# fpthink/EPC-Net

Measured on AMD Instinct MI355X. Metric: point-clouds/sec (4096 pts) descriptor extraction, higher is better.
Workload: dtype f16x3; 1 GPU; epc-net inference, batch 64x4096x3 fp32 per GPU, NetVLAD K=64, 256-D output (BASELINE.json configs[1]); num_points=4096, precision=EPC_PRECISION_F32 (include/epcnet.h), weights=seeded random init of the architecture (no checkpoint payloads exist), parallelism=independent clouds sharded over 1 GPU(s), no data-path collective

## Files before the change

epc-net_amd/csrc/block.hip:

```cpp
#include "train_common.h"

#define BLK_WAVES 12
#define BLK_THREADS (64 * BLK_WAVES)
#define BLK_PERSIST_MAX_ROUNDS 4096
#define ST_STRIDE 68
#define BLK_PACK EPC_BLOCK_PACK_FLOATS
#define BLK_PACK_S EPC_BLOCK_PACK_FLOATS_S
#define BLK_LDS_FLOATS (BLK_PACK_S + BLK_WAVES * 32 * ST_STRIDE)


__device__ __forceinline__ void acc_init_bias(f32x16& acc, const float* bias32, int h) {
#pragma unroll
    for (int g = 0; g < 4; ++g) {
        const float4 b = ld4(bias32 + 8 * g + 4 * h);
        acc[4 * g + 0] = b.x;
        acc[4 * g + 1] = b.y;
        acc[4 * g + 2] = b.z;
        acc[4 * g + 3] = b.w;
    }
}

__device__ __forceinline__ void kahan_add(float& sum, float& comp, float v) {
    const float y = v - comp;
    const float t = sum + y;
    comp = (t - sum) - y;
    sum = t;
}

__device__ __forceinline__ void relu16(f32x16& a) {
#pragma unroll
    for (int r = 0; r < 16; ++r) a[r] = fmaxf(a[r], 0.f);
}


__device__ __forceinline__ f16x8 ldfrag_h(const float* p) {
    return __builtin_bit_cast(f16x8, *reinterpret_cast<const u32x4*>(p));
}
__device__ __forceinline__ void layer_s64(const float* lw, const float* lbias, const float* ltinv, const f16x8 (&bh)[4],
                                          const f16x8 (&bl)[4], float inv_row, f32x16 (&acc)[2], int lane) {
    const int h = lane >> 5;
#pragma unroll
    for (int t = 0; t < 2; ++t) {
#pragma unroll
        for (int r = 0; r < 16; ++r) acc[t][r] = 0.f;
#pragma unroll
        for (int s = 0; s < 4; ++s) {
            const f16x8 ah = ldfrag_h(lw + (((t * 4 + s) * 2 + 0) * 64 + lane) * 4);
            const f16x8 al = ldfrag_h(lw + (((t * 4 + s) * 2 + 1) * 64 + lane) * 4);
            acc[t] = mfma_f16(al, bh[s], acc[t]);
            acc[t] = mfma_f16(ah, bl[s], acc[t]);
            acc[t] = mfma_f16(ah, bh[s], acc[t]);
        }
#pragma unroll
        for (int g = 0; g < 4; ++g) {
            const float4 ti = ld4(ltinv + 32 * t + 8 * g + 4 * h), b = ld4(lbias + 32 * t + 8 * g + 4 * h);
            acc[t][4 * g + 0] = __builtin_fmaf(acc[t][4 * g + 0], inv_row * ti.x, b.x);
            acc[t][4 * g + 1] = __builtin_fmaf(acc[t][4 * g + 1], inv_row * ti.y, b.y);
            acc[t][4 * g + 2] = __builtin_fmaf(acc[t][4 * g + 2], inv_row * ti.z, b.z);
            acc[t][4 * g + 3] = __builtin_fmaf(acc[t][4 * g + 3], inv_row * ti.w, b.w);
        }
    }
}

__device__ __forceinline__ void layer_acc64(const float* lw, const float* lbias, const float* ltinv, const f32x16 (&in)[2],
                                            f32x16 (&acc)[2], int lane) {
    float m = 0.f;
#pragma unroll
    for (int t = 0; t < 2; ++t)
#pragma unroll
        for (int r = 0; r < 16; ++r) m = fmaxf(m, fabsf(in[t][r]));
    m = fmaxf(m, __shfl_xor(m, 32));
    float sc, inv_row;
    row_scale_pow2(m, sc, inv_row);
    f16x8 fh[4], fl[4];
#pragma unroll
    for (int st = 0; st < 4; ++st) {
        float v[8];
#pragma unroll
        for (int q = 0; q < 8; ++q) v[q] = in[st >> 1][8 * (st & 1) + q];
        split8_f16s(v, sc, fh[st], fl[st]);
    }
    layer_s64(lw, lbias, ltinv, fh, fl, inv_row, acc, lane);
}

__device__ __forceinline__ void acc_to_stage(float* st, const f32x16 (&acc)[2], int lane) {
    const int j = lane & 31, h = lane >> 5;
#pragma unroll
    for (int t = 0; t < 2; ++t)
#pragma unroll
        for (int g = 0; g < 4; ++g)
            st4(st + j * ST_STRIDE + 32 * t + 8 * g + 4 * h,
                make_float4(acc[t][4 * g], acc[t][4 * g + 1], acc[t][4 * g + 2], acc[t][4 * g + 3]));
}

__device__ __forceinline__ float stage_to_bop(const float* st, f16x8 (&bh)[4], f16x8 (&bl)[4], int lane) {
    const int j = lane & 31, h = lane >> 5;
    float v[4][8];
    float m = 0.f;
#pragma unroll
    for (int s = 0; s < 4; ++s) {
        const float4 a = ld4(st + j * ST_STRIDE + 16 * s + 8 * h), b = ld4(st + j * ST_STRIDE + 16 * s + 8 * h + 4);
        v[s][0] = a.x, v[s][1] = a.y, v[s][2] = a.z, v[s][3] = a.w, v[s][4] = b.x, v[s][5] = b.y, v[s][6] = b.z, v[s][7] = b.w;
#pragma unroll
        for (int q = 0; q < 8; ++q) m = fmaxf(m, fabsf(v[s][q]));
    }
    m = fmaxf(m, __shfl_xor(m, 32));
    float sc, inv_row;
    row_scale_pow2(m, sc, inv_row);
#pragma unroll
    for (int s = 0; s < 4; ++s) split8_f16s(v[s], sc, bh[s], bl[s]);
    return inv_row;
}

__device__ __forceinline__ void load_nb20(const char* lists, unsigned row, int cap, bool u16, int (&nb)[EPC_KNN_SELECT]) {
    static_assert(EPC_KNN_SELECT == 20, "five int4 / two int4 + one int2 per row");
    if (u16) {
        const char* r = lists + (size_t)row * cap * 2;
        const uint4 a = *reinterpret_cast<const uint4*>(r), b = *reinterpret_cast<const uint4*>(r + 16);
        const uint2 c = *reinterpret_cast<const uint2*>(r + 32);
        const unsigned int w[10] = {a.x, a.y, a.z, a.w, b.x, b.y, b.z, b.w, c.x, c.y};
#pragma unroll
        for (int k = 0; k < 10; ++k) {
            nb[2 * k] = (int)(w[k] & 0xffffu);
            nb[2 * k + 1] = (int)(w[k] >> 16);
        }
    } else {
        const int4* il = reinterpret_cast<const int4*>(lists + (size_t)row * cap * 4);
#pragma unroll
        for (int m4 = 0; m4 < EPC_KNN_SELECT / 4; ++m4) {
            const int4 t = il[m4];
            nb[4 * m4] = t.x;
            nb[4 * m4 + 1] = t.y;
            nb[4 * m4 + 2] = t.z;
            nb[4 * m4 + 3] = t.w;
        }
    }
}
__device__ __forceinline__ int list_entry(const void* lists, size_t slot, bool u16) {
    return u16 ? (int)reinterpret_cast<const unsigned short*>(lists)[slot] : reinterpret_cast<const int32_t*>(lists)[slot];
}

__global__ __launch_bounds__(BLK_THREADS) void proxyconv_block_kernel(
    const float* __restrict__ x, const float* __restrict__ xyz, const void* __restrict__ idx, int idx_u16,
    const int32_t* __restrict__ cnt, const float* __restrict__ kth, int cap, const float* __restrict__ pack,
    int has_next, int total_points, int n, float kdiv, float* __restrict__ out, int out_stride, int out_off,
    float* __restrict__ x_next) {
    extern __shared__ __attribute__((aligned(16))) float lds[];
    __shared__ int s_next_tile;
    const int tid = threadIdx.x, lane = tid & 63, wave = tid >> 6;
    if (tid == 0) s_next_tile = 0;
    for (int o = tid * 4; o < BLK_PACK_S; o += BLK_THREADS * 4) st4(lds + o, ld4(pack + o));
    __syncthreads();
    const float* wa = lds;
    const float* ba = lds + 4096;
    const float* wb = lds + 4160;
    const float* bb = lds + 4160 + 4096;
    const float* wn = lds + 8320;
    const float* bn = lds + 8320 + 4096;
    const float* tia = lds + BLK_PACK;
    const float* tib = tia + 64;
    const float* tin = tia + 128;
    float* st = lds + BLK_PACK_S + wave * 32 * ST_STRIDE;

    const int ntiles = total_points / 32;
    const int nwg = (int)gridDim.x, per = ntiles / nwg, rem = ntiles % nwg;
    auto first_tile_of = [&](int wg) { return wg * per + min(wg, rem); };
    const int xq = nwg >> 3, xr = nwg & 7, xcd = (int)blockIdx.x & 7, slot = (int)blockIdx.x >> 3;
    const int xcd_wgs = xq + (xcd < xr ? 1 : 0);
    const int xcd_first = xcd < xr ? xcd * (xq + 1) : xr * (xq + 1) + (xcd - xr) * xq;
    const int t_begin = first_tile_of(xcd_first), t_end = first_tile_of(xcd_first + xcd_wgs);
    const int p = lane >> 4, q = lane & 15;
    const bool u16 = idx_u16 != 0;
    const float rk = 1.0f / kdiv;
    auto div_k = [&](float a) {
        const float q0 = a * rk;
        return __builtin_fmaf(__builtin_fmaf(-q0, kdiv, a), rk, q0);
    };
  for (;;) {
    int t_draw = 0;
    if (lane == 0) t_draw = atomicAdd(&s_next_tile, 1);
    const int d = __builtin_amdgcn_readfirstlane(t_draw);
    const int tile = t_begin + (d >> 2) * (xcd_wgs * 4) + slot * 4 + (d & 3);
    if (tile >= t_end) break;
    const int g0 = tile * 32;
    const int cloud_base = __builtin_amdgcn_readfirstlane((g0 / n) * n);
    const char* xc = reinterpret_cast<const char*>(x) + (size_t)cloud_base * 256;
    auto row32 = [&](int row) { return *reinterpret_cast<const float4*>(xc + (unsigned)(row * 256 + q * 16)); };
    const int wg0 = __builtin_amdgcn_readfirstlane(g0);

    float4 xm[8];
#pragma unroll
    for (int s = 0; s < 8; ++s) {
        const int g = g0 + 4 * s + p;
        const int c = cnt[g];
        const bool ovf = c > cap;
        float4 acc = make_float4(0.f, 0.f, 0.f, 0.f);
        if (!ovf) {
            int nb[EPC_KNN_SELECT];
            load_nb20(reinterpret_cast<const char*>(idx), (unsigned)(wg0 + 4 * s + p), cap, u16, nb);
            float4 v[EPC_KNN_SELECT];
#pragma unroll
            for (int m = 0; m < EPC_KNN_SELECT; ++m) v[m] = row32(nb[m]);
#pragma unroll
            for (int m = 0; m < EPC_KNN_SELECT; ++m) {
                acc.x += v[m].x;
                acc.y += v[m].y;
                acc.z += v[m].z;
                acc.w += v[m].w;
            }
            for (int m = EPC_KNN_SELECT; m < c; ++m) {
                const float4 w = row32(list_entry(idx, (size_t)g * cap + m, u16));
                acc.x += w.x;
                acc.y += w.y;
                acc.z += w.z;
                acc.w += w.w;
            }
        }
        if (__any(ovf)) {
            if (ovf) {
                const float* pc = xyz + (size_t)cloud_base * 3;
                const int i = g - cloud_base;
                const float xi = pc[3 * i], yi = pc[3 * i + 1], zi = pc[3 * i + 2];
                const float sqi = sq3(xi, yi, zi);
                const float kv = kth[g];
                float4 comp = make_float4(0.f, 0.f, 0.f, 0.f);
                for (int j = 0; j < n; ++j) {
                    const float xj = pc[3 * j], yj = pc[3 * j + 1], zj = pc[3 * j + 2];
                    const float a = neg_sq_dist(sqi, xi, yi, zi, xj, yj, zj, sq3(xj, yj, zj));
                    if (a >= kv) {
                        const float4 w = row32(j);
                        kahan_add(acc.x, comp.x, w.x);
                        kahan_add(acc.y, comp.y, w.y);
                        kahan_add(acc.z, comp.z, w.z);
                        kahan_add(acc.w, comp.w, w.w);
                    }
                }
            }
        }
        acc.x = div_k(acc.x), acc.y = div_k(acc.y), acc.z = div_k(acc.z), acc.w = div_k(acc.w);
        xm[s] = acc;
        const float4 xi4 = row32(g - cloud_base);
        st4(st + (4 * s + p) * ST_STRIDE + 4 * q,
            make_float4(acc.x - xi4.x, acc.y - xi4.y, acc.z - xi4.z, acc.w - xi4.w));
    }

    f16x8 bh[4], bl[4];
    f32x16 a1[2], a2[2];
    float inv_row = stage_to_bop(st, bh, bl, lane);
    layer_s64(wa, ba, tia, bh, bl, inv_row, a1, lane);
    relu16(a1[0]);
    relu16(a1[1]);
    layer_acc64(wb, bb, tib, a1, a2, lane);
    relu16(a2[0]);
    relu16(a2[1]);

    acc_to_stage(st, a2, lane);
#pragma unroll
    for (int s = 0; s < 8; ++s) {
        float* row = st + (4 * s + p) * ST_STRIDE + 4 * q;
        const float4 t = ld4(row);
        const float4 o = make_float4(t.x + xm[s].x, t.y + xm[s].y, t.z + xm[s].z, t.w + xm[s].w);
        st4(out + (size_t)(g0 + 4 * s + p) * out_stride + out_off + 4 * q, o);
        st4(row, o);
    }
    if (!has_next) continue;

    inv_row = stage_to_bop(st, bh, bl, lane);
    layer_s64(wn, bn, tin, bh, bl, inv_row, a1, lane);
    relu16(a1[0]);
    relu16(a1[1]);
    acc_to_stage(st, a1, lane);
#pragma unroll
    for (int s = 0; s < 8; ++s)
        st4(x_next + (size_t)(g0 + 4 * s + p) * 64 + 4 * q, ld4(st + (4 * s + p) * ST_STRIDE + 4 * q));
  }
}

#define ST16 72


__device__ __forceinline__ void layer_f16(const float* lw, const float* lbias, const f16x8 (&bop)[4], f32x16 (&acc)[2],
                                          int lane) {
    const int h = lane >> 5;
#pragma unroll
    for (int t = 0; t < 2; ++t) {
        acc_init_bias(acc[t], lbias + 32 * t, h);
#pragma unroll
        for (int s = 0; s < 4; ++s) {
            const f16x8 ah = ldfrag16(lw + (((t * 4 + s) * 2 + 0) * 64 + lane) * 4);
            const f16x8 al = ldfrag16(lw + (((t * 4 + s) * 2 + 1) * 64 + lane) * 4);
            acc[t] = mfma_f16(al, bop[s], acc[t]);
            acc[t] = mfma_f16(ah, bop[s], acc[t]);
        }
    }
}

typedef unsigned short u16x2_t __attribute__((ext_vector_type(2)));
__device__ __forceinline__ void range_track(u16x2_t& m, unsigned int packed_pair) {
    m = __builtin_elementwise_max(m, __builtin_bit_cast(u16x2_t, packed_pair & 0x7fff7fffu));
}
__device__ __forceinline__ void range_track4(u16x2_t& m, const u32x4& w) {
    range_track(m, w[0]), range_track(m, w[1]), range_track(m, w[2]), range_track(m, w[3]);
}

__device__ __forceinline__ uint2 relu_descale_pack4(const f32x16& a, int r0) {
    _Float16 hv[4];
#pragma unroll
    for (int e = 0; e < 4; ++e) hv[e] = (_Float16)(fmaxf(a[r0 + e], 0.f) * (1.0f / W5_SCALE));
    uint2 w;
    w.x = (unsigned)__builtin_bit_cast(unsigned short, hv[0]) | ((unsigned)__builtin_bit_cast(unsigned short, hv[1]) << 16);
    w.y = (unsigned)__builtin_bit_cast(unsigned short, hv[2]) | ((unsigned)__builtin_bit_cast(unsigned short, hv[3]) << 16);
    return w;
}

__device__ __forceinline__ void acc_to_stage16(unsigned short* st, const f32x16 (&acc)[2], int lane) {
    const int j = lane & 31, h = lane >> 5;
#pragma unroll
    for (int t = 0; t < 2; ++t)
#pragma unroll
        for (int g = 0; g < 4; ++g)
            *reinterpret_cast<uint2*>(st + j * ST16 + 32 * t + 8 * g + 4 * h) = relu_descale_pack4(acc[t], 4 * g);
}

__device__ __forceinline__ void stage16_to_bop(const unsigned short* st, f16x8 (&bop)[4], int lane) {
    const int j = lane & 31, h = lane >> 5;
#pragma unroll
    for (int s = 0; s < 4; ++s)
        bop[s] = __builtin_bit_cast(f16x8, *reinterpret_cast<const u32x4*>(st + j * ST16 + 16 * s + 8 * h));
}

#define BLK16_WAVES 16
#define BLK16_THREADS (64 * BLK16_WAVES)
#define BLK16_LDS_BYTES (BLK_PACK * 4 + BLK16_WAVES * 32 * ST16 * 2)

__global__ __launch_bounds__(BLK16_THREADS) void proxyconv_block_f16_kernel(
    const unsigned short* __restrict__ x16, const float* __restrict__ xyz, const void* __restrict__ idx, int idx_u16,
    const int32_t* __restrict__ cnt, const float* __restrict__ kth, int cap, const float* __restrict__ pack,
    int has_next, int total_points, int n, float kdiv, unsigned short* __restrict__ out16, int out_stride, int out_off,
    unsigned short* __restrict__ x_next16, int32_t* __restrict__ status) {
    extern __shared__ __attribute__((aligned(16))) float lds[];
    const int tid = threadIdx.x, lane = tid & 63, wave = tid >> 6;
    for (int o = tid * 4; o < BLK_PACK; o += BLK16_THREADS * 4) st4(lds + o, ld4(pack + o));
    __syncthreads();
    const float* wa = lds;
    const float* ba = lds + 4096;
    const float* wb = lds + 4160;
    const float* bb = lds + 4160 + 4096;
    const float* wn = lds + 8320;
    const float* bn = lds + 8320 + 4096;
    unsigned short* st = reinterpret_cast<unsigned short*>(lds + BLK_PACK) + wave * 32 * ST16;

    const int bid = xcd_contiguous_block(blockIdx.x, gridDim.x);
    const int g0 = (bid * BLK16_WAVES + wave) * 32;
    if (g0 >= total_points) return;
    const int cloud_base = __builtin_amdgcn_readfirstlane((g0 / n) * n);
    const int p = lane >> 3, q = lane & 7;
    const char* xc = reinterpret_cast<const char*>(x16) + (size_t)cloud_base * 128;
    auto row16 = [&](int row) { return *reinterpret_cast<const u32x4*>(xc + (unsigned)(row * 128 + q * 16)); };
    auto add_row = [&](float (&acc)[8], const u32x4& raw) {
#pragma unroll
        for (int w2 = 0; w2 < 4; ++w2) {
            asm("v_fma_mix_f32 %0, %1, 1.0, %0 op_sel:[0,0,0] op_sel_hi:[1,0,0]" : "+v"(acc[2 * w2]) : "v"(raw[w2]));
            asm("v_fma_mix_f32 %0, %1, 1.0, %0 op_sel:[1,0,0] op_sel_hi:[1,0,0]" : "+v"(acc[2 * w2 + 1]) : "v"(raw[w2]));
        }
    };
    const int wg0 = __builtin_amdgcn_readfirstlane(g0);
    const bool u16 = idx_u16 != 0;
    const float rk = 1.0f / kdiv;
    auto div_k = [&](float a) {
        const float q0 = a * rk;
        return __builtin_fmaf(__builtin_fmaf(-q0, kdiv, a), rk, q0);
    };

    u16x2_t rmax = {0, 0};
    auto report_range = [&]() {
        const bool over = max(rmax[0], rmax[1]) >= 0x7c00;
        if (status && __builtin_amdgcn_ballot_w64(over) != 0ull && lane == 0) atomicOr(status + g0 / n, EPC_STATUS_FP16_RANGE);
    };
    float xm[4][8];
#pragma unroll
    for (int s = 0; s < 4; ++s) {
        const int g = g0 + 8 * s + p;
        const int c = cnt[g];
        const bool ovf = c > cap;
        float acc[8];
#pragma unroll
        for (int e = 0; e < 8; ++e) acc[e] = 0.f;
        if (!ovf) {
            int nb[EPC_KNN_SELECT];
            load_nb20(reinterpret_cast<const char*>(idx), (unsigned)(wg0 + 8 * s + p), cap, u16, nb);
            u32x4 raw[EPC_KNN_SELECT];
#pragma unroll
            for (int m = 0; m < EPC_KNN_SELECT; ++m) raw[m] = row16(nb[m]);
#pragma unroll
            for (int m = 0; m < EPC_KNN_SELECT; ++m) add_row(acc, raw[m]);
            for (int m = EPC_KNN_SELECT; m < c; ++m) add_row(acc, row16(list_entry(idx, (size_t)g * cap + m, u16)));
        }
        if (__any(ovf)) {
            if (ovf) {
                const float* pc = xyz + (size_t)cloud_base * 3;
                const int i = g - cloud_base;
                const float xi = pc[3 * i], yi = pc[3 * i + 1], zi = pc[3 * i + 2];
                const float sqi = sq3(xi, yi, zi);
                const float kv = kth[g];
                for (int j = 0; j < n; ++j) {
                    const float xj = pc[3 * j], yj = pc[3 * j + 1], zj = pc[3 * j + 2];
                    const float a = neg_sq_dist(sqi, xi, yi, zi, xj, yj, zj, sq3(xj, yj, zj));
                    if (a >= kv) add_row(acc, row16(j));
                }
            }
        }
        const f16x8 self = __builtin_bit_cast(f16x8, row16(g - cloud_base));
        f16x8 t16;
#pragma unroll
        for (int e = 0; e < 8; ++e) {
            xm[s][e] = div_k(acc[e]);
            t16[e] = (_Float16)(xm[s][e] - (float)self[e]);
        }
        const u32x4 tw = __builtin_bit_cast(u32x4, t16);
        range_track4(rmax, tw);
        *reinterpret_cast<u32x4*>(st + (8 * s + p) * ST16 + 8 * q) = tw;
    }

    f16x8 bop[4];
    f32x16 a1[2], a2[2];
    stage16_to_bop(st, bop, lane);
    layer_f16(wa, ba, bop, a1, lane);
    {
#pragma unroll
        for (int k4 = 0; k4 < 4; ++k4) {
            const uint2 lo = relu_descale_pack4(a1[k4 >> 1], 8 * (k4 & 1)), hi = relu_descale_pack4(a1[k4 >> 1], 8 * (k4 & 1) + 4);
            u32x4 w;
            w[0] = lo.x, w[1] = lo.y, w[2] = hi.x, w[3] = hi.y;
            range_track4(rmax, w);
            bop[k4] = __builtin_bit_cast(f16x8, w);
        }
    }
    layer_f16(wb, bb, bop, a2, lane);

    acc_to_stage16(st, a2, lane);
#pragma unroll
    for (int s = 0; s < 4; ++s) {
        unsigned short* row = st + (8 * s + p) * ST16 + 8 * q;
        const u32x4 t16w = *reinterpret_cast<const u32x4*>(row);
        const f16x8 t16 = __builtin_bit_cast(f16x8, t16w);
        f16x8 o16;
#pragma unroll
        for (int e = 0; e < 8; ++e) o16[e] = (_Float16)((float)t16[e] + xm[s][e]);
        const u32x4 ow = __builtin_bit_cast(u32x4, o16);
        range_track4(rmax, t16w);
        range_track4(rmax, ow);
        *reinterpret_cast<u32x4*>(out16 + (size_t)(g0 + 8 * s + p) * out_stride + out_off + 8 * q) = ow;
        *reinterpret_cast<u32x4*>(row) = ow;
    }
    if (!has_next) {
        report_range();
        return;
    }

    stage16_to_bop(st, bop, lane);
    layer_f16(wn, bn, bop, a1, lane);
    acc_to_stage16(st, a1, lane);
#pragma unroll
    for (int s = 0; s < 4; ++s) {
        const u32x4 xw = *reinterpret_cast<const u32x4*>(st + (8 * s + p) * ST16 + 8 * q);
        range_track4(rmax, xw);
        *reinterpret_cast<u32x4*>(x_next16 + (size_t)(g0 + 8 * s + p) * 64 + 8 * q) = xw;
    }
    report_range();
}

__global__ __launch_bounds__(256) void conv1_kernel(const float* __restrict__ xyz, const float* __restrict__ pack,
                                                    int total_points, float* __restrict__ x,
                                                    unsigned short* __restrict__ x16, int32_t* __restrict__ status,
                                                    int n) {
    const int t = blockIdx.x * 256 + threadIdx.x;
    const int g = t >> 4, q = t & 15;
    if (g >= total_points) return;
    const float px = xyz[3 * (size_t)g], py = xyz[3 * (size_t)g + 1], pz = xyz[3 * (size_t)g + 2];
    const float4 w0 = ld4(pack + 4 * q), w1 = ld4(pack + 64 + 4 * q), w2 = ld4(pack + 128 + 4 * q);
    const float4 b = ld4(pack + 192 + 4 * q);
    const float4 y = conv1_quad(px, py, pz, w0, w1, w2, b);
    if (x) st4(x + (size_t)g * 64 + 4 * q, y);
    if (x16) {
        reinterpret_cast<uint2*>(x16)[(size_t)g * 16 + q] = pack_half4(y);
        if (status && fmaxf(fmaxf(y.x, y.y), fmaxf(y.z, y.w)) > 65504.0f) atomicOr(status + g / n, EPC_STATUS_FP16_RANGE);
    }
}

int epc_conv1_launch(const float* xyz, const void* packed_conv1, int num_points_total, float* x, void* x16,
                     int32_t* status, int n, void* stream) {
    EPC_CHECK_ARG(xyz && packed_conv1 && (x || x16), "null pointer");
    EPC_CHECK_ARG(num_points_total >= 0 && (!status || n > 0), "bad shape");
    if (num_points_total == 0) return EPC_OK;
    const long threads = (long)num_points_total * 16;
    hipLaunchKernelGGL(conv1_kernel, dim3((unsigned)((threads + 255) / 256)), dim3(256), 0, (hipStream_t)stream,
                       xyz, (const float*)packed_conv1, num_points_total, x, (unsigned short*)x16, status, n);
    EPC_CHECK_LAUNCH();
    return EPC_OK;
}

extern "C" int epc_conv1_fwd(const float* xyz, const void* packed_conv1, int num_points_total, float* x, void* x16,
                             void* stream) {
    return epc_conv1_launch(xyz, packed_conv1, num_points_total, x, x16, nullptr, 0, stream);
}

extern "C" int epc_proxyconv_block_fwd(const float* x, const void* x16, const float* xyz, const void* idx, int idx_u16,
                                       const int32_t* cnt, const float* kth, int cap, const void* packed_block,
                                       int has_next, int num_clouds, int n, int knn, float* out, void* out16,
                                       int out_stride, int out_off, float* x_next, void* x_next16, int32_t* status,
                                       void* stream) {
    const bool f16 = x16 != nullptr;
    EPC_CHECK_ARG(xyz && idx && cnt && kth && packed_block, "null pointer");
    if (f16) {
        EPC_CHECK_ARG(out16 && (!has_next || x_next16), "fp16 mode needs out16 (and x_next16 when has_next)");
        EPC_CHECK_ARG(out_stride % 8 == 0 && out_off % 8 == 0 && out_off + 64 <= out_stride, "bad output slice");
    } else {
        EPC_CHECK_ARG(x && out && (!has_next || x_next), "f32 mode needs x, out (and x_next when has_next)");
        EPC_CHECK_ARG(out_stride % 4 == 0 && out_off % 4 == 0 && out_off + 64 <= out_stride, "bad output slice");
    }
    EPC_CHECK_ARG(cap == EPC_KNN_CAP, "neighbour-list capacity must be EPC_KNN_CAP (32)");
    EPC_CHECK_ARG(n > 0 && n % 32 == 0, "num_points must be a multiple of 32");
    EPC_CHECK_ARG(knn > 0, "KNN divisor must be positive");
    if (num_clouds <= 0) return num_clouds == 0 ? EPC_OK : EPC_EINVAL;
    const long total = (long)num_clouds * n;
    EPC_CHECK_ARG(total < (1L << 31), "too many points");
    const size_t lds_bytes = f16 ? (size_t)BLK16_LDS_BYTES : BLK_LDS_FLOATS * sizeof(float);
    const void* fn = f16 ? reinterpret_cast<const void*>(proxyconv_block_f16_kernel)
                         : reinterpret_cast<const void*>(proxyconv_block_kernel);
    EPC_SET_DYN_LDS(fn, lds_bytes);
    const int wpb = f16 ? BLK16_WAVES : BLK_WAVES;
    unsigned blocks = (unsigned)((total + wpb * 32 - 1) / (wpb * 32));
    if (!f16) {
        const int num_cus = epc_device_cu_count();
        if (blocks > (unsigned)num_cus && blocks <= (unsigned)BLK_PERSIST_MAX_ROUNDS * (unsigned)num_cus) blocks = (unsigned)num_cus;
    }
    if (f16)
        hipLaunchKernelGGL(proxyconv_block_f16_kernel, dim3(blocks), dim3(BLK16_THREADS), lds_bytes, (hipStream_t)stream,
                           (const unsigned short*)x16, xyz, idx, idx_u16, cnt, kth, cap, (const float*)packed_block, has_next,
                           (int)total, n, (float)knn, (unsigned short*)out16, out_stride, out_off,
                           (unsigned short*)x_next16, status);
    else
        hipLaunchKernelGGL(proxyconv_block_kernel, dim3(blocks), dim3(BLK_THREADS), lds_bytes, (hipStream_t)stream, x,
                           xyz, idx, idx_u16, cnt, kth, cap, (const float*)packed_block, has_next, (int)total, n, (float)knn,
                           out, out_stride, out_off, x_next);
    EPC_CHECK_LAUNCH();
    return EPC_OK;
}
```

epc-net_amd/lib.py:

```python
from __future__ import annotations

import ctypes
import os
import re
from ctypes import POINTER, c_char_p, c_float, c_int, c_int32, c_void_p

import torch

_HERE = os.path.dirname(os.path.abspath(__file__))
LIB_PATH = os.environ.get("EPCNET_LIB") or os.path.join(_HERE, "libepcnet_hip.so")
HEADER_PATH = os.path.join(os.path.dirname(_HERE), "include", "epcnet.h")

_SCALARS = {"int": c_int, "long": ctypes.c_long, "long long": ctypes.c_longlong, "float": c_float,
            "size_t": ctypes.c_size_t, "int32_t": c_int32, "uint32_t": ctypes.c_uint32}
_REVISIT_SCALARS = dict(_SCALARS, double=ctypes.c_double)
_POINTEES = {"float*": torch.float32, "double*": torch.float64, "int32_t*": torch.int32, "int*": torch.int32, "long*": torch.int64}


def parse_header(text: str, need_status: bool = True, scalars=_SCALARS):
    text = re.sub(r"/\*.*?\*/", " ", text, flags=re.S)
    text = re.sub(r"#ifdef __cplusplus.*?#endif", " ", text, flags=re.S)
    constants = {n: int(v, 0) for n, v in re.findall(r"^[ \t]*#[ \t]*define[ \t]+(EPC_\w+)[ \t]+(.*?)[ \t]*$", text, flags=re.M)}
    enum = re.search(r"typedef\s+enum\s+epc_status\s*\{(.*?)\}", text, flags=re.S)
    if not enum and need_status:
        raise ValueError("epcnet.h: no enum epc_status")
    status = {n.strip(): int(v, 0) for n, v in (m.split("=") for m in enum.group(1).split(","))} if enum else {}
    text = re.sub(r"^[ \t]*#.*$", " ", text, flags=re.M)
    text = re.sub(r"typedef\s+(struct|enum)\s+\w+\s*(\{[^{}]*\})?\s*\w+\s*;", " ", text)

    def ctype(t):
        return re.sub(r"\s*\*\s*", "*", " ".join(re.sub(r"\bconst\b", " ", t).split()))

    functions = {}
    for decl in text.split(";"):
        if not decl.strip():
            continue
        m = re.fullmatch(r"\s*([\w\s*]+?)\b(epc(?:net)?_\w+)\s*\((.*)\)\s*", decl, flags=re.S)
        if not m or m.group(2) in functions:
            raise ValueError("epcnet.h: not a declaration, or a second one of its name: %r" % " ".join(decl.split()))
        ret, name, params, names = ctype(m.group(1)), m.group(2), [], []
        if ret not in scalars and ret != "char*":
            raise ValueError("epcnet.h: %s: unknown return type %r" % (name, ret))
        for p in ([] if m.group(3).strip() == "void" else m.group(3).split(",")):
            pm = re.fullmatch(r"\s*(.*[\s*])(\w+)\s*", p, flags=re.S)
            if not pm or (ctype(pm.group(1)) not in scalars and "*" not in pm.group(1)):
                raise ValueError("epcnet.h: %s: unknown parameter type in %r" % (name, " ".join(p.split())))
            params.append(ctype(pm.group(1)))
            names.append(pm.group(2))
        functions[name] = (ret, params, names)
    return functions, constants, status


if not os.path.exists(HEADER_PATH):
    raise ImportError(
        "%s is missing: the binding is derived from the library's header (keep include/ beside the package).  "
        "There is no second copy of the declarations." % HEADER_PATH)
with open(HEADER_PATH) as _f:
    _functions, _constants, _status = parse_header(_f.read())
POSES_HEADER_PATH = os.path.join(os.path.dirname(HEADER_PATH), "epcnet_poses.h")
if not os.path.exists(POSES_HEADER_PATH):
    raise ImportError("%s is missing: the binding of the pose entries is derived from it" % POSES_HEADER_PATH)
with open(POSES_HEADER_PATH) as _f:
    _pose_functions, _pose_constants, _ = parse_header(_f.read(), need_status=False)
if set(_pose_functions) & set(_functions) or set(_pose_constants) & set(_constants):
    raise ImportError("epcnet_poses.h declares a name epcnet.h declares")
_constants.update(_pose_constants)
POSE_EXPORTS = list(_pose_functions)
SCANS_HEADER_PATH = os.path.join(os.path.dirname(HEADER_PATH), "epcnet_scans.h")
if not os.path.exists(SCANS_HEADER_PATH):
    raise ImportError("%s is missing: the binding of the scan entries is derived from it" % SCANS_HEADER_PATH)
with open(SCANS_HEADER_PATH) as _f:
    _scan_functions, _scan_constants, _ = parse_header(_f.read(), need_status=False)
if set(_scan_functions) & (set(_functions) | set(_pose_functions)) or set(_scan_constants) & set(_constants):
    raise ImportError("epcnet_scans.h declares a name epcnet.h or epcnet_poses.h declares")
_constants.update(_scan_constants)
SCAN_EXPORTS = list(_scan_functions)
SUBMAPS_HEADER_PATH = os.path.join(os.path.dirname(HEADER_PATH), "epcnet_submaps.h")
if not os.path.exists(SUBMAPS_HEADER_PATH):
    raise ImportError("%s is missing: the binding of the submap entries is derived from it" % SUBMAPS_HEADER_PATH)
with open(SUBMAPS_HEADER_PATH) as _f:
    _submap_functions, _submap_constants, _ = parse_header(_f.read(), need_status=False)
if (set(_submap_functions) & (set(_functions) | set(_pose_functions) | set(_scan_functions))
        or set(_submap_constants) & set(_constants)):
    raise ImportError("epcnet_submaps.h declares a name an earlier header declares")
_constants.update(_submap_constants)
SUBMAP_EXPORTS = list(_submap_functions)
STAMPS_HEADER_PATH = os.path.join(os.path.dirname(HEADER_PATH), "epcnet_stamps.h")
if not os.path.exists(STAMPS_HEADER_PATH):
    raise ImportError("%s is missing: the binding of the stamp entries is derived from it" % STAMPS_HEADER_PATH)
with open(STAMPS_HEADER_PATH) as _f:
    _stamp_functions, _stamp_constants, _ = parse_header(_f.read(), need_status=False)
if (set(_stamp_functions) & (set(_functions) | set(_pose_functions) | set(_scan_functions) | set(_submap_functions))
        or set(_stamp_constants) & set(_constants)):
    raise ImportError("epcnet_stamps.h declares a name an earlier header declares")
_constants.update(_stamp_constants)
STAMP_EXPORTS = list(_stamp_functions)
REVISITS_HEADER_PATH = os.path.join(os.path.dirname(HEADER_PATH), "epcnet_revisits.h")
if not os.path.exists(REVISITS_HEADER_PATH):
    raise ImportError("%s is missing: the binding of the revisit entries is derived from it" % REVISITS_HEADER_PATH)
with open(REVISITS_HEADER_PATH) as _f:
    _revisit_functions, _revisit_constants, _ = parse_header(_f.read(), need_status=False, scalars=_REVISIT_SCALARS)
if (set(_revisit_functions) & (set(_functions) | set(_pose_functions) | set(_scan_functions) | set(_submap_functions) | set(_stamp_functions))
        or set(_revisit_constants) & set(_constants)):
    raise ImportError("epcnet_revisits.h declares a name an earlier header declares")
_constants.update(_revisit_constants)
REVISIT_EXPORTS = list(_revisit_functions)
PAIRS_HEADER_PATH = os.path.join(os.path.dirname(HEADER_PATH), "epcnet_pairs.h")
if not os.path.exists(PAIRS_HEADER_PATH):
    raise ImportError("%s is missing: the binding of the pair entries is derived from it" % PAIRS_HEADER_PATH)
with open(PAIRS_HEADER_PATH) as _f:
    _pair_functions, _pair_constants, _ = parse_header(_f.read(), need_status=False, scalars=_REVISIT_SCALARS)
if (set(_pair_functions) & (set(_functions) | set(_pose_functions) | set(_scan_functions) | set(_submap_functions) | set(_stamp_functions)
                            | set(_revisit_functions))
        or set(_pair_constants) & set(_constants)):
    raise ImportError("epcnet_pairs.h declares a name an earlier header declares")
_constants.update(_pair_constants)
PAIR_EXPORTS = list(_pair_functions)
globals().update(_constants, **_status)
EXPORTS = list(_functions)
STATUS_NAMES = {v: n for n, v in _status.items()}
PRECISION_IDS = {"f32": _constants["EPC_PRECISION_F32"], "fast": _constants["EPC_PRECISION_FAST"]}
STAGE_NAMES = ["sort", "knn", "conv1", "block1", "block2", "block3", "block4", "conv5", "aggregate", "head"]
assert len(STAGE_NAMES) == _constants["EPC_NUM_STAGES"]


class EpcNetError(RuntimeError):
    def __init__(self, status: int, message: str):
        super().__init__("%s (%d): %s" % (STATUS_NAMES.get(status, "?"), status, message))
        self.status = status


class EpcCfg(ctypes.Structure):
    _fields_ = [("arch", c_int32), ("num_points", c_int32), ("input_dim", c_int32), ("knn", c_int32),
                ("cluster_size", c_int32), ("output_dim", c_int32), ("groups", c_int32),
                ("micro_batch", c_int32), ("precision", c_int32)]


_P = c_void_p


class ChainFwdBlock(ctypes.Structure):
    _fields_ = [(n, _P) for n in ("gamma0", "beta0", "in_bias", "Wa", "ba", "gamma_a", "beta_a", "Wb", "bb", "gamma_b", "beta_b",
                                  "W0_next", "b0_next", "z0", "mean0", "var0", "mean_a", "var_a", "mean_b", "var_b",
                                  "d", "za", "zb", "z0_next")]


class ChainFwdArgs(ctypes.Structure):
    _fields_ = [("blk", ChainFwdBlock * _constants["EPC_CHAIN_MAX_BLOCKS"]), ("nblocks", c_int), ("xyz", _P), ("idx", _P), ("cnt", _P),
                ("kth", _P), ("cap", c_int), ("num_clouds", c_int), ("n", c_int), ("knn", c_int), ("cat", _P), ("cat_bf16", _P),
                ("eps", c_float), ("workspace", _P), ("spin_ticks", ctypes.c_longlong)]


if not os.path.exists(LIB_PATH):
    raise ImportError(
        "%s is missing: build the HIP extension first (python -c 'import __graft_entry__ as g; g.build()' or "
        "make -C epc-net_amd/csrc).  There is no CPU fallback." % LIB_PATH)

_lib = ctypes.CDLL(LIB_PATH)

_POINTERS = {"epc_cfg*": POINTER(EpcCfg), "epc_chain_fwd_args*": POINTER(ChainFwdArgs)}
for _name, (_ret, _params, _) in (list(_functions.items()) + list(_pose_functions.items()) + list(_scan_functions.items())
                                  + list(_submap_functions.items()) + list(_stamp_functions.items()) + list(_revisit_functions.items())
                                  + list(_pair_functions.items())):
    _fn = getattr(_lib, _name)
    _fn.restype = c_char_p if _ret == "char*" else _REVISIT_SCALARS[_ret]
    _fn.argtypes = [_REVISIT_SCALARS.get(_t) or _POINTERS.get(_t, c_void_p) for _t in _params]


def lib() -> ctypes.CDLL:
    return _lib


def check(status: int) -> None:
    if status != _status["EPC_OK"]:
        raise EpcNetError(status, (_lib.epc_last_error() or b"").decode("utf-8", "replace"))


def ptr(t) -> int:
    if t is None:
        return None
    if not t.is_cuda:
        raise EpcNetError(-1, "tensor must live on a ROCm device: the HIP path has no CPU fallback")
    if not t.is_contiguous():
        raise EpcNetError(-1, "tensor must be contiguous")
    return t.data_ptr()


def micro_batch_of(cfg: "EpcCfg", num_clouds: int) -> int:
    mb = cfg.micro_batch if cfg.micro_batch > 0 else (64 if cfg.arch == _constants["EPC_ARCH_EPC_NET"] else 256)
    return max(1, min(int(num_clouds), int(mb)))


def current_stream() -> int:
    return torch.cuda.current_stream().cuda_stream


def _converter(where: str, ctype: str):
    if "*" in ctype:
        dtype = _POINTEES.get(ctype)

        def pointer(a):
            if a is None:
                return None
            try:
                on_device = a.is_cuda
            except AttributeError:
                return a
            if not on_device:
                raise EpcNetError(-1, "%s: tensor must live on a ROCm device: the HIP path has no CPU fallback" % where)
            if dtype is not None and a.dtype is not dtype:
                raise EpcNetError(-1, "%s: the header declares %s there, the tensor is %s" % (where, dtype, a.dtype))
            return a.data_ptr()
        return pointer
    cast = float if ctype in ("float", "double") else int

    def scalar(a):
        if type(a) is cast:
            return a
        if isinstance(a, torch.Tensor):
            raise TypeError("%s: a tensor where the header declares a scalar" % where)
        return cast(a)
    return scalar


def _launcher(name: str, fn, types, names):
    signature = "%s(%s)" % (name, ", ".join("%s %s" % tn for tn in zip(types, names)))
    converters = [_converter("%s: argument %d (%s %s)" % (name, i + 1, t, n), t) for i, (t, n) in enumerate(zip(types[:-1], names))]
    ok = _status["EPC_OK"]

    def launch(*args, stream=None):
        if len(args) != len(converters):
            raise TypeError("%s takes %d arguments and the stream, got %d" % (signature, len(converters), len(args)))
        status = fn(*[c(a) for c, a in zip(converters, args)], current_stream() if stream is None else stream)
        if status != ok:
            check(status)
    launch.__name__ = launch.__qualname__ = name
    launch.__doc__ = signature
    return launch


class run:
    """The checked call form of every LAUNCHING entry point -- one whose last parameter is ``void* stream`` -- by name:
    ``run.epc_col_sum(dy, rows, cout, db, ws, n)`` takes the header's arguments without the stream.  A tensor is legal at a pointer
    parameter only, must live on the device and have the dtype of a typed pointee (``_POINTEES``; anything goes at ``void*``); its
    address is passed, strides are the caller's.  None, an int address and ctypes objects pass unchanged, scalars through int() /
    float().  The stream is the current one (or ``stream=``), the returned status goes through ``check``.  Everything else --
    size queries, ``*_ok``, the forwards whose stream is not last -- is called on the raw handle ``lib()``."""


LAUNCHING = [_n for _n, (_, _t, _pn) in _functions.items() if _t and (_t[-1], _pn[-1]) == ("void*", "stream")]
for _name in LAUNCHING:
    assert _functions[_name][0] == "int", "%s takes a stream and does not return a status" % _name
    setattr(run, _name, staticmethod(_launcher(_name, getattr(_lib, _name), *_functions[_name][1:])))
for _name, (_ret, _t, _pn) in _pose_functions.items():
    assert _ret == "int" and (_t[-1], _pn[-1]) == ("void*", "stream"), "%s does not take a stream last and return a status" % _name
    setattr(run, _name, staticmethod(_launcher(_name, getattr(_lib, _name), _t, _pn)))
for _name, (_ret, _t, _pn) in (list(_scan_functions.items()) + list(_submap_functions.items()) + list(_stamp_functions.items())
                               + list(_revisit_functions.items()) + list(_pair_functions.items())):
    if _t and (_t[-1], _pn[-1]) == ("void*", "stream"):
        assert _ret == "int", "%s takes a stream and does not return a status" % _name
        setattr(run, _name, staticmethod(_launcher(_name, getattr(_lib, _name), _t, _pn)))


def require_gpu() -> None:
    if not torch.cuda.is_available():
        raise EpcNetError(-3, "no ROCm device visible: the EPC-Net HIP path cannot run (no CPU fallback)")
```

Before: 59120 clouds/s.

## Add fast neighbor-gather path with coalesced index staging and software-pipelined gathers

Adds a templated fast path to the fp32 proxy-conv block kernel. When the cap matches the compile-time value and no point in the tile overflows, it loads the tile's neighbor index lists with coalesced wave-wide uint4 loads, parks them in LDS, and software-pipelines the 20-neighbor row gathers so the next row's loads overlap the current sum. Output stores become nontemporal. The old path remains as form 0 behind a new entry point, which adds code size and register pressure.

```diff
diff --git a/epc-net_amd/csrc/block.hip b/epc-net_amd/csrc/block.hip
--- a/epc-net_amd/csrc/block.hip
+++ b/epc-net_amd/csrc/block.hip
@@ -1,4 +1,6 @@
+#include <type_traits>
 #include "train_common.h"
+#include "../../include/epcnet_forms.h"
 
 #define BLK_WAVES 12
 #define BLK_THREADS (64 * BLK_WAVES)
@@ -27,6 +29,12 @@
     sum = t;
 }
 
+__device__ __forceinline__ void st4_stream(float* p, float4 v) {
+    typedef float f32x4_t __attribute__((ext_vector_type(4)));
+    const f32x4_t w = {v.x, v.y, v.z, v.w};
+    __builtin_nontemporal_store(w, reinterpret_cast<f32x4_t*>(p));
+}
+
 __device__ __forceinline__ void relu16(f32x16& a) {
 #pragma unroll
     for (int r = 0; r < 16; ++r) a[r] = fmaxf(a[r], 0.f);
@@ -140,6 +148,30 @@
     return u16 ? (int)reinterpret_cast<const unsigned short*>(lists)[slot] : reinterpret_cast<const int32_t*>(lists)[slot];
 }
 
+template <bool U16>
+struct Nb20Words {
+    unsigned int w[U16 ? EPC_KNN_SELECT / 2 : EPC_KNN_SELECT];
+    __device__ __forceinline__ void load(const float* row) {
+        static_assert(EPC_KNN_SELECT == 20, "five uint4 / two uint4 + one uint2 per row");
+        const uint4* r = reinterpret_cast<const uint4*>(row);
+        if (U16) {
+            const uint4 a = r[0], b = r[1];
+            const uint2 c = *reinterpret_cast<const uint2*>(row + 8);
+            w[0] = a.x, w[1] = a.y, w[2] = a.z, w[3] = a.w, w[4] = b.x, w[5] = b.y, w[6] = b.z, w[7] = b.w, w[8] = c.x, w[9] = c.y;
+        } else {
+#pragma unroll
+            for (int m4 = 0; m4 < EPC_KNN_SELECT / 4; ++m4) {
+                const uint4 t = r[m4];
+                w[4 * m4] = t.x, w[4 * m4 + 1] = t.y, w[4 * m4 + 2] = t.z, w[4 * m4 + 3] = t.w;
+            }
+        }
+    }
+    __device__ __forceinline__ int entry(int m) const {
+        return U16 ? (int)((m & 1) ? w[m >> 1] >> 16 : w[m >> 1] & 0xffffu) : (int)w[m];
+    }
+};
+
+template <int FORM>
 __global__ __launch_bounds__(BLK_THREADS) void proxyconv_block_kernel(
     const float* __restrict__ x, const float* __restrict__ xyz, const void* __restrict__ idx, int idx_u16,
     const int32_t* __restrict__ cnt, const float* __restrict__ kth, int cap, const float* __restrict__ pack,
@@ -176,6 +208,7 @@
         const float q0 = a * rk;
         return __builtin_fmaf(__builtin_fmaf(-q0, kdiv, a), rk, q0);
     };
+    const bool cap_ok = cap == EPC_KNN_CAP;
   for (;;) {
     int t_draw = 0;
     if (lane == 0) t_draw = atomicAdd(&s_next_tile, 1);
@@ -189,6 +222,68 @@
     const int wg0 = __builtin_amdgcn_readfirstlane(g0);
 
     float4 xm[8];
+    int c32 = 0;
+    uint4 l0 = make_uint4(0, 0, 0, 0), l1 = l0;
+    const uint4* lb = reinterpret_cast<const uint4*>(reinterpret_cast<const char*>(idx) +
+                                                     (size_t)tile * (32 * EPC_KNN_CAP) * (u16 ? 2 : 4));
+    if (FORM == 1 && cap_ok) {
+        c32 = cnt[g0 + (lane & 31)];
+        l0 = lb[lane];
+        l1 = lb[64 + lane];
+    }
+    const bool fast = FORM == 1 && cap_ok && !__any(c32 > EPC_KNN_SELECT);
+    auto park = [&](int i, const uint4& w, int rb) {
+        *reinterpret_cast<uint4*>(st + (16 * i / rb) * ST_STRIDE + (16 * i % rb) / 4) = w;
+    };
+    auto fast_passes = [&](auto u16_c) {
+        constexpr bool U16 = decltype(u16_c)::value;
+        constexpr int rb = (U16 ? 2 : 4) * EPC_KNN_CAP;
+        uint4 l2 = l0, l3 = l0;
+        if (!U16) {
+            l2 = lb[128 + lane];
+            l3 = lb[192 + lane];
+        }
+        park(lane, l0, rb);
+        park(64 + lane, l1, rb);
+        Nb20Words<U16> nb;
+        float4 v[EPC_KNN_SELECT];
+        nb.load(st + p * ST_STRIDE);
+        float4 own = row32(g0 + p - cloud_base);
+#pragma unroll
+        for (int m = 0; m < EPC_KNN_SELECT; ++m) v[m] = row32(nb.entry(m));
+        if (!U16) {
+            park(128 + lane, l2, rb);
+            park(192 + lane, l3, rb);
+        }
+#pragma unroll
+        for (int s = 0; s < 8; ++s) {
+            float4 own_n = own;
+            if (s < 7) {
+                nb.load(st + (4 * (s + 1) + p) * ST_STRIDE);
+                own_n = row32(g0 + 4 * (s + 1) + p - cloud_base);
+            }
+            float4 acc = make_float4(0.f, 0.f, 0.f, 0.f);
+#pragma unroll
+            for (int m = 0; m < EPC_KNN_SELECT; ++m) {
+                acc.x += v[m].x;
+                acc.y += v[m].y;
+                acc.z += v[m].z;
+                acc.w += v[m].w;
+                if (s < 7) v[m] = row32(nb.entry(m));
+            }
+            acc.x = div_k(acc.x), acc.y = div_k(acc.y), acc.z = div_k(acc.z), acc.w = div_k(acc.w);
+            xm[s] = acc;
+            st4(st + (4 * s + p) * ST_STRIDE + 4 * q,
+                make_float4(acc.x - own.x, acc.y - own.y, acc.z - own.z, acc.w - own.w));
+            own = own_n;
+        }
+    };
+    if (fast) {
+        if (u16)
+            fast_passes(std::true_type{});
+        else
+            fast_passes(std::false_type{});
+    } else {
 #pragma unroll
     for (int s = 0; s < 8; ++s) {
         const int g = g0 + 4 * s + p;
@@ -243,6 +338,7 @@
         st4(st + (4 * s + p) * ST_STRIDE + 4 * q,
             make_float4(acc.x - xi4.x, acc.y - xi4.y, acc.z - xi4.z, acc.w - xi4.w));
     }
+    }
 
     f16x8 bh[4], bl[4];
     f32x16 a1[2], a2[2];
@@ -260,7 +356,7 @@
         float* row = st + (4 * s + p) * ST_STRIDE + 4 * q;
         const float4 t = ld4(row);
         const float4 o = make_float4(t.x + xm[s].x, t.y + xm[s].y, t.z + xm[s].z, t.w + xm[s].w);
-        st4(out + (size_t)(g0 + 4 * s + p) * out_stride + out_off + 4 * q, o);
+        st4_stream(out + (size_t)(g0 + 4 * s + p) * out_stride + out_off + 4 * q, o);
         st4(row, o);
     }
     if (!has_next) continue;
@@ -505,11 +601,11 @@
     return epc_conv1_launch(xyz, packed_conv1, num_points_total, x, x16, nullptr, 0, stream);
 }
 
-extern "C" int epc_proxyconv_block_fwd(const float* x, const void* x16, const float* xyz, const void* idx, int idx_u16,
-                                       const int32_t* cnt, const float* kth, int cap, const void* packed_block,
-                                       int has_next, int num_clouds, int n, int knn, float* out, void* out16,
-                                       int out_stride, int out_off, float* x_next, void* x_next16, int32_t* status,
-                                       void* stream) {
+static int proxyconv_block_fwd_impl(const float* x, const void* x16, const float* xyz, const void* idx, int idx_u16,
+                                    const int32_t* cnt, const float* kth, int cap, const void* packed_block,
+                                    int has_next, int num_clouds, int n, int knn, float* out, void* out16,
+                                    int out_stride, int out_off, float* x_next, void* x_next16, int32_t* status,
+                                    int form, void* stream) {
     const bool f16 = x16 != nullptr;
     EPC_CHECK_ARG(xyz && idx && cnt && kth && packed_block, "null pointer");
     if (f16) {
@@ -526,8 +622,9 @@
     const long total = (long)num_clouds * n;
     EPC_CHECK_ARG(total < (1L << 31), "too many points");
     const size_t lds_bytes = f16 ? (size_t)BLK16_LDS_BYTES : BLK_LDS_FLOATS * sizeof(float);
+    const auto f32_kernel = form == 0 ? proxyconv_block_kernel<0> : proxyconv_block_kernel<1>;
     const void* fn = f16 ? reinterpret_cast<const void*>(proxyconv_block_f16_kernel)
-                         : reinterpret_cast<const void*>(proxyconv_block_kernel);
+                         : reinterpret_cast<const void*>(f32_kernel);
     EPC_SET_DYN_LDS(fn, lds_bytes);
     const int wpb = f16 ? BLK16_WAVES : BLK_WAVES;
     unsigned blocks = (unsigned)((total + wpb * 32 - 1) / (wpb * 32));
@@ -541,9 +638,27 @@
                            (int)total, n, (float)knn, (unsigned short*)out16, out_stride, out_off,
                            (unsigned short*)x_next16, status);
     else
-        hipLaunchKernelGGL(proxyconv_block_kernel, dim3(blocks), dim3(BLK_THREADS), lds_bytes, (hipStream_t)stream, x,
+        hipLaunchKernelGGL(f32_kernel, dim3(blocks), dim3(BLK_THREADS), lds_bytes, (hipStream_t)stream, x,
                            xyz, idx, idx_u16, cnt, kth, cap, (const float*)packed_block, has_next, (int)total, n, (float)knn,
                            out, out_stride, out_off, x_next);
     EPC_CHECK_LAUNCH();
     return EPC_OK;
 }
+
+extern "C" int epc_proxyconv_block_fwd(const float* x, const void* x16, const float* xyz, const void* idx, int idx_u16,
+                                       const int32_t* cnt, const float* kth, int cap, const void* packed_block,
+                                       int has_next, int num_clouds, int n, int knn, float* out, void* out16,
+                                       int out_stride, int out_off, float* x_next, void* x_next16, int32_t* status,
+                                       void* stream) {
+    return proxyconv_block_fwd_impl(x, x16, xyz, idx, idx_u16, cnt, kth, cap, packed_block, has_next, num_clouds, n, knn, out,
+                                    out16, out_stride, out_off, x_next, x_next16, status, 1, stream);
+}
+
+extern "C" int epcnet_block_fwd_form(const float* x, const void* x16, const float* xyz, const void* idx, int idx_u16,
+                                     const int32_t* cnt, const float* kth, int cap, const void* packed_block, int has_next,
+                                     int num_clouds, int n, int knn, float* out, void* out16, int out_stride, int out_off,
+                                     float* x_next, void* x_next16, int32_t* status, int form, void* stream) {
+    EPC_CHECK_ARG(form == 0 || form == 1, "form 0 or 1");
+    return proxyconv_block_fwd_impl(x, x16, xyz, idx, idx_u16, cnt, kth, cap, packed_block, has_next, num_clouds, n, knn, out,
+                                    out16, out_stride, out_off, x_next, x_next16, status, form, stream);
+}
diff --git a/epc-net_amd/lib.py b/epc-net_amd/lib.py
--- a/epc-net_amd/lib.py
+++ b/epc-net_amd/lib.py
@@ -116,6 +116,17 @@
     raise ImportError("epcnet_pairs.h declares a name an earlier header declares")
 _constants.update(_pair_constants)
 PAIR_EXPORTS = list(_pair_functions)
+FORMS_HEADER_PATH = os.path.join(os.path.dirname(HEADER_PATH), "epcnet_forms.h")
+if not os.path.exists(FORMS_HEADER_PATH):
+    raise ImportError("%s is missing: the binding of the form entries is derived from it" % FORMS_HEADER_PATH)
+with open(FORMS_HEADER_PATH) as _f:
+    _form_functions, _form_constants, _ = parse_header(_f.read(), need_status=False)
+if (set(_form_functions) & (set(_functions) | set(_pose_functions) | set(_scan_functions) | set(_submap_functions) | set(_stamp_functions)
+                            | set(_revisit_functions) | set(_pair_functions))
+        or set(_form_constants) & set(_constants)):
+    raise ImportError("epcnet_forms.h declares a name an earlier header declares")
+_constants.update(_form_constants)
+FORM_EXPORTS = list(_form_functions)
 globals().update(_constants, **_status)
 EXPORTS = list(_functions)
 STATUS_NAMES = {v: n for n, v in _status.items()}
@@ -161,7 +172,7 @@
 _POINTERS = {"epc_cfg*": POINTER(EpcCfg), "epc_chain_fwd_args*": POINTER(ChainFwdArgs)}
 for _name, (_ret, _params, _) in (list(_functions.items()) + list(_pose_functions.items()) + list(_scan_functions.items())
                                   + list(_submap_functions.items()) + list(_stamp_functions.items()) + list(_revisit_functions.items())
-                                  + list(_pair_functions.items())):
+                                  + list(_pair_functions.items()) + list(_form_functions.items())):
     _fn = getattr(_lib, _name)
     _fn.restype = c_char_p if _ret == "char*" else _REVISIT_SCALARS[_ret]
     _fn.argtypes = [_REVISIT_SCALARS.get(_t) or _POINTERS.get(_t, c_void_p) for _t in _params]
@@ -256,7 +267,7 @@
     assert _ret == "int" and (_t[-1], _pn[-1]) == ("void*", "stream"), "%s does not take a stream last and return a status" % _name
     setattr(run, _name, staticmethod(_launcher(_name, getattr(_lib, _name), _t, _pn)))
 for _name, (_ret, _t, _pn) in (list(_scan_functions.items()) + list(_submap_functions.items()) + list(_stamp_functions.items())
-                               + list(_revisit_functions.items()) + list(_pair_functions.items())):
+                               + list(_revisit_functions.items()) + list(_pair_functions.items()) + list(_form_functions.items())):
     if _t and (_t[-1], _pn[-1]) == ("void*", "stream"):
         assert _ret == "int", "%s takes a stream and does not return a status" % _name
         setattr(run, _name, staticmethod(_launcher(_name, getattr(_lib, _name), _t, _pn)))
diff --git a/include/epcnet_forms.h b/include/epcnet_forms.h
--- /dev/null
+++ b/include/epcnet_forms.h
@@ -0,0 +1,19 @@
+#ifndef EPCNET_FORMS_H
+#define EPCNET_FORMS_H
+
+#include <stddef.h>
+#include <stdint.h>
+
+#ifdef __cplusplus
+extern "C" {
+#endif
+
+int epcnet_block_fwd_form(const float* x, const void* x16, const float* xyz, const void* idx, int idx_u16, const int32_t* cnt,
+                          const float* kth, int cap, const void* packed_block, int has_next, int num_clouds, int n, int knn,
+                          float* out, void* out16, int out_stride, int out_off, float* x_next, void* x_next16, int32_t* status,
+                          int form, void* stream);
+
+#ifdef __cplusplus
+}
+#endif
+#endif
```

After: 62560 clouds/s (median of 6 runs). 5.8% higher.
